# Chuanming-Liu/DAzimSurfTomo

Measured on AMD Instinct MI355X. Metric: FMM traveltime fields/sec (256^2 grid, 16 periods) + LSQR SpMV HBM GB/s, higher is better.
Workload: dtype f32

## Files before the change

dazimsurftomo_amd/csrc/disp.hip:

```cpp
#include <cmath>

#include "dazim_internal.h"

namespace {

constexpr int NL = 200;
constexpr int NP = 60;
constexpr int NZMAX = 64;
constexpr int DT = 256;
constexpr int TW = 64;
constexpr int TEAM = 16;
constexpr int NEVN = 11;

struct Layer {
  double tmp;
  float d;
  float rfac;
  float fm, den;
  int iv;
  float rden;
};

struct DispArgs {
  int ncol, nz, kmax, nvar, mmax;
  int team;
  int var0, nvarp;
  const float *vel;
  const Layer *lay;
  const double *t;
  float *cg;
  int ngroup, nchunk, pchunk;
  unsigned *counter;
  int *ready;
  double *st_c;
  double *st_d;
  int *st_f;
  int ffwd;
  int exp3;
  unsigned *ff_stat;
  int *ff_m;
  double *ff_c;
  int *ff_v;
  double *svs, *svp, *srho;
  double *pv;
  int *nfail;
};

__device__ __forceinline__ double sgn(double x) { return copysign(1.0, x); }

__device__ __forceinline__ double frcp(double b) {
  double r = __builtin_amdgcn_rcp(b);
  r = __builtin_fma(__builtin_fma(-b, r, 1.0), r, r);
  r = __builtin_fma(__builtin_fma(-b, r, 1.0), r, r);
  return r;
}
__device__ __forceinline__ double fdiv(double a, double b) {
  const double r = frcp(b);
  const double q = a * r;
  return __builtin_fma(__builtin_fma(-b, q, a), r, q);
}

__device__ __forceinline__ double fsqrt(double x, double &rs) {
  const double y = __builtin_amdgcn_rsq(x);
  double g = x * y, h = 0.5 * y;
  double r = __builtin_fma(-h, g, 0.5);
  g = __builtin_fma(g, r, g);
  h = __builtin_fma(h, r, h);
  r = __builtin_fma(-g, g, x);
  g = __builtin_fma(r, h, g);
  r = __builtin_fma(-h, g, 0.5);
  h = __builtin_fma(h, r, h);
  rs = h + h;
  return x > 0.0 ? g : 0.0;
}

struct Knots {
  const float *vs, *vp, *rho;
  int pi, pq;
  float pv;
  __device__ __forceinline__ float get(int q, int i) const {
    const float *b = q == 0 ? vs : (q == 1 ? vp : rho);
    const float v = b[i - 1];
    return (i == pi && q == pq) ? pv : v;
  }
};

template <int RDEN>
__device__ __forceinline__ void layer_model(const Knots &K, const Layer *lay, int m, int nz, bool fast, float &a,
                                            float &b, float &rho, float &d) {
  const Layer L = lay[m - 1];
  float rvp, rvs, rrho;
  if (L.iv > 0) {
    const int i = L.iv;
    const float p0 = K.get(1, i), p1 = K.get(1, i + 1);
    const float s0 = K.get(0, i), s1 = K.get(0, i + 1);
    const float r0 = K.get(2, i), r1 = K.get(2, i + 1);
    if (RDEN == 1) {
      rvp = p0 + L.fm * (p1 - p0) * L.rden;
      rvs = s0 + L.fm * (s1 - s0) * L.rden;
      rrho = r0 + L.fm * (r1 - r0) * L.rden;
    } else if (RDEN == 2 && fast) {
      const float tp = L.fm * (p1 - p0), ts = L.fm * (s1 - s0), tr = L.fm * (r1 - r0);
      float qp = tp * L.rden, qs = ts * L.rden, qr = tr * L.rden;
      qp = __builtin_fmaf(__builtin_fmaf(-L.den, qp, tp), L.rden, qp);
      qs = __builtin_fmaf(__builtin_fmaf(-L.den, qs, ts), L.rden, qs);
      qr = __builtin_fmaf(__builtin_fmaf(-L.den, qr, tr), L.rden, qr);
      rvp = p0 + qp;
      rvs = s0 + qs;
      rrho = r0 + qr;
    } else {
      rvp = p0 + L.fm * (p1 - p0) / L.den;
      rvs = s0 + L.fm * (s1 - s0) / L.den;
      rrho = r0 + L.fm * (r1 - r0) / L.den;
    }
  } else {
    rvp = K.get(1, nz);
    rvs = K.get(0, nz);
    rrho = K.get(2, nz);
  }
  a = (float)((double)rvp * L.tmp);
  b = (float)((double)rvs * L.tmp);
  rho = rrho * L.rfac;
  d = L.d;
}

template <int RDEN>
__device__ double dltar4(const Knots &K, const Layer *lay, int mmax, int nz, bool fast, double wvno, double omga, bool exp3 = false) {
#pragma clang fp contract(fast)
  double e0, e1, e2, e3, e4;
  double omega = omga;
  if (omega < 1.0e-4) omega = 1.0e-4;
  const double wvno2 = wvno * wvno;
  const double romega = 1.0 / omega;
  float fa, fb, frho, fd;
  layer_model<RDEN>(K, lay, mmax, nz, fast, fa, fb, frho, fd);
  {
    const double xka = omega / (double)fa, xkb = omega / (double)fb;
    double wvnop = wvno + xka, wvnom = fabs(wvno - xka);
    const double ra = sqrt(wvnop * wvnom);
    wvnop = wvno + xkb;
    wvnom = fabs(wvno - xkb);
    const double rb = sqrt(wvnop * wvnom);
    const double t = (double)fb / omega;
    const double gammk = 2.0 * t * t;
    const double gam = gammk * wvno2;
    const double gamm1 = gam - 1.0;
    const double rho1 = (double)frho;
    e0 = rho1 * rho1 * (gamm1 * gamm1 - gam * gammk * ra * rb);
    e1 = -rho1 * ra;
    e2 = rho1 * (gamm1 - gammk * ra * rb);
    e3 = rho1 * rb;
    e4 = wvno2 - ra * rb;
  }
  for (int m = mmax - 1; m >= 1; m--) {
    layer_model<RDEN>(K, lay, m, nz, fast, fa, fb, frho, fd);
    const double xka = fdiv(omega, (double)fa), xkb = fdiv(omega, (double)fb);
    const double t = (double)fb * romega;
    const double gammk = 2.0 * t * t;
    const double gam = gammk * wvno2;
    double wvnop = wvno + xka, wvnom = fabs(wvno - xka);
    double rra;
    const double ra = fsqrt(wvnop * wvnom, rra);
    wvnop = wvno + xkb;
    wvnom = fabs(wvno - xkb);
    double rrb;
    const double rb = fsqrt(wvnop * wvnom, rrb);
    const double dpth = (double)fd, rho1 = (double)frho;
    const double rrho1 = frcp(rho1), rrho2 = rrho1 * rrho1;
    const double p = ra * dpth, q = rb * dpth;
    double w, x, y, z, cosp, cosq, sinp, sinq, fac, pex = 0.0, sex = 0.0;
    if (wvno > xka) pex = p;
    if (wvno > xkb) sex = q;
    const double ep = pex > 0.0 ? exp(-pex) : 1.0, eq = sex > 0.0 ? exp(-sex) : 1.0;
    if (wvno < xka) {
      sincos(p, &sinp, &cosp);
      w = sinp * rra;
      x = -ra * sinp;
    } else if (wvno == xka) {
      cosp = 1.0;
      w = dpth;
      x = 0.0;
    } else {
      fac = 0.0;
      if (p < 16) fac = exp3 ? exp(-2.0 * p) : ep * ep;
      cosp = (1.0 + fac) * 0.5;
      sinp = (1.0 - fac) * 0.5;
      w = sinp * rra;
      x = ra * sinp;
    }
    if (wvno < xkb) {
      sincos(q, &sinq, &cosq);
      y = sinq * rrb;
      z = -rb * sinq;
    } else if (wvno == xkb) {
      cosq = 1.0;
      y = dpth;
      z = 0.0;
    } else {
      fac = 0.0;
      if (q < 16) fac = exp3 ? exp(-2.0 * q) : eq * eq;
      cosq = (1.0 + fac) * 0.5;
      sinq = (1.0 - fac) * 0.5;
      y = sinq * rrb;
      z = rb * sinq;
    }
    const double exa = pex + sex;
    double a0 = 0.0;
    if (exa < 60.0) a0 = exp3 ? exp(-exa) : ep * eq;
    const double cpcq = cosp * cosq, cpy = cosp * y, cpz = cosp * z, cqw = cosq * w, cqx = cosq * x;
    const double xy = x * y, xz = x * z, wy = w * y, wz = w * z;
    const double gamm1 = gam - 1.0;
    const double twgm1 = gam + gamm1, gmgmk = gam * gammk, gmgm1 = gam * gamm1, gm1sq = gamm1 * gamm1;
    const double rho2 = rho1 * rho1, a0pq = a0 - cpcq;
    const double ca11 = cpcq - 2.0 * gmgm1 * a0pq - gmgmk * xz - wvno2 * gm1sq * wy;
    const double ca12 = (wvno2 * cpy - cqx) * rrho1;
    const double ca13 = -(twgm1 * a0pq + gammk * xz + wvno2 * gamm1 * wy) * rrho1;
    const double ca14 = (cpz - wvno2 * cqw) * rrho1;
    const double ca15 = -(2.0 * wvno2 * a0pq + xz + wvno2 * wvno2 * wy) * rrho2;
    const double ca21 = (gmgmk * cpz - gm1sq * cqw) * rho1;
    const double ca22 = cpcq;
    const double ca23 = gammk * cpz - gamm1 * cqw;
    const double ca24 = -wz;
    const double ca25 = ca14;
    const double ca41 = (gm1sq * cpy - gmgmk * cqx) * rho1;
    const double ca42 = -xy;
    const double ca43 = gamm1 * cpy - gammk * cqx;
    const double ca44 = ca22;
    const double ca45 = ca12;
    const double ca51 = -(2.0 * gmgmk * gm1sq * a0pq + gmgmk * gmgmk * xz + gm1sq * gm1sq * wy) * rho2;
    const double ca52 = ca41;
    const double ca53 = -(gammk * gamm1 * twgm1 * a0pq + gam * gammk * gammk * xz + gamm1 * gm1sq * wy) * rho1;
    const double ca54 = ca21;
    const double ca55 = ca11;
    const double tt = -2.0 * wvno2;
    const double ca31 = tt * ca53, ca32 = tt * ca43, ca33 = a0 + 2.0 * (cpcq - ca11), ca34 = tt * ca23,
                 ca35 = tt * ca13;
    double n0 = 0.0 + e0 * ca11;  n0 = n0 + e1 * ca21;  n0 = n0 + e2 * ca31;  n0 = n0 + e3 * ca41;  n0 = n0 + e4 * ca51;
    double n1 = 0.0 + e0 * ca12;  n1 = n1 + e1 * ca22;  n1 = n1 + e2 * ca32;  n1 = n1 + e3 * ca42;  n1 = n1 + e4 * ca52;
    double n2 = 0.0 + e0 * ca13;  n2 = n2 + e1 * ca23;  n2 = n2 + e2 * ca33;  n2 = n2 + e3 * ca43;  n2 = n2 + e4 * ca53;
    double n3 = 0.0 + e0 * ca14;  n3 = n3 + e1 * ca24;  n3 = n3 + e2 * ca34;  n3 = n3 + e3 * ca44;  n3 = n3 + e4 * ca54;
    double n4 = 0.0 + e0 * ca15;  n4 = n4 + e1 * ca25;  n4 = n4 + e2 * ca35;  n4 = n4 + e3 * ca45;  n4 = n4 + e4 * ca55;
    double t1 = fmax(fmax(fmax(fabs(n0), fabs(n1)), fmax(fabs(n2), fabs(n3))), fabs(n4));
    if (t1 < 1.e-40) t1 = 1.0;
    const double r1 = frcp(t1);
    e0 = n0 * r1;
    e1 = n1 * r1;
    e2 = n2 * r1;
    e3 = n3 * r1;
    e4 = n4 * r1;
  }
  return e0;
}

__device__ float gtsolh(float a, float b) {
  float c = 0.95f * b;
  for (int i = 0; i < 5; i++) {
    const float gamma = b / a;
    const float kappa = c / b;
    const float k2 = kappa * kappa;
    const float gk2 = (gamma * kappa) * (gamma * kappa);
    const float fac1 = sqrtf(1.0f - gk2);
    const float fac2 = sqrtf(1.0f - k2);
    const float fr = (2.0f - k2) * (2.0f - k2) - 4.0f * fac1 * fac2;
    float frp = -4.0f * (2.0f - k2) * kappa + 4.0f * fac2 * gamma * gamma * kappa / fac1 + 4.0f * fac1 * kappa / fac2;
    frp = frp / b;
    c = c - fr / frp;
  }
  return c;
}

__device__ __forceinline__ void brocher(float vs, float &vp, float &rho) {
  const float v2 = vs * vs, v3 = v2 * vs, v4 = v3 * vs;
  const float p = 0.9409f + 2.0947f * vs - 0.8206f * v2 + 0.2683f * v3 - 0.0251f * v4;
  const float p2 = p * p, p3 = p2 * p, p4 = p3 * p, p5 = p4 * p;
  vp = p;
  rho = 1.6612f * p - 0.4721f * p2 + 0.0671f * p3 - 0.0043f * p4 + 0.000106f * p5;
}

enum { P_G1, P_G2, P_N0, P_NA, P_NB, P_GV, P_GW, P_DONE };

template <int RDEN>
__device__ __forceinline__ void startup(const Knots &K, const Layer *lay, int mmax, int nz, bool fast, float &betmx, float &cc1) {
  float betmn = 1.e20f, a_mn = 1.0f, b_mn = 1.0f;
  betmx = -1.e20f;
  int jsol = 1;
  for (int m = 1; m <= mmax; m++) {
    float fa, fb, fr, fd;
    layer_model<RDEN>(K, lay, m, nz, fast, fa, fb, fr, fd);
    if (fb > 0.01f && fb < betmn) {
      betmn = fb;
      a_mn = fa;
      b_mn = fb;
      jsol = 1;
    } else if (fb <= 0.01f && fa < betmn) {
      betmn = fa;
      a_mn = fa;
      b_mn = fb;
      jsol = 0;
    }
    if (fb > betmx) betmx = fb;
  }
  cc1 = jsol == 0 ? betmn : gtsolh(a_mn, b_mn);
  cc1 = .95f * cc1;
  cc1 = .90f * cc1;
}

constexpr int FF_BLOCKS = 8;
constexpr double FF_MARGIN = 0.02;
constexpr float FF_MAXDROP = 0.25f;
template <int RDEN>
__global__ __launch_bounds__(64) void disp_bracket_kernel(DispArgs A) {
  __shared__ Layer s_lay[NL];
  __shared__ float s_knot[3 * NZMAX];
  const int lane = threadIdx.x, col = blockIdx.x;
  const int nz = A.nz, mmax = A.mmax;
  for (int i = lane; i < mmax; i += 64) s_lay[i] = A.lay[i];
  for (int k = lane; k < nz; k += 64) {
    const float vs = A.vel[(size_t)k * A.ncol + col];
    float vp, rho;
    brocher(vs, vp, rho);
    s_knot[k] = vs;
    s_knot[nz + k] = vp;
    s_knot[2 * nz + k] = rho;
  }
  __syncthreads();
  Knots K;
  K.vs = s_knot;
  K.vp = s_knot + nz;
  K.rho = s_knot + 2 * nz;
  K.pi = 0;
  K.pq = -1;
  K.pv = 0.0f;
  bool fast = false;
  if (RDEN == 2) {
    bool ok = true;
    for (int i = 1; i < nz; i++)
#pragma unroll
      for (int q = 0; q < 3; q++) {
        const float ad = fabsf(K.get(q, i + 1) - K.get(q, i));
        ok = ok && (ad == 0.0f || (ad >= 1.0e-30f && ad <= 1.0e28f));
      }
    fast = __all(ok);
  }
  float betmx, cc1;
  startup<RDEN>(K, s_lay, mmax, nz, fast, betmx, cc1);
  const double dc = fabs((double)0.005f), TWOPI = 2.0 * 3.141592653589793;
  const double omega = TWOPI / A.t[0];
  const double climit = (double)betmx + dc;
  double cblk = (double)cc1;
  unsigned long long prev_last = 0;
  int found = 0;
  double cfound = 0.0, clast_prev = 0.0;
  double alast_prev = 0.0;
  int jfirst = -1;
  bool wiggle = false;
  for (int blk = 0; blk < FF_BLOCKS; blk++) {
    double c = cblk;
    for (int i = 0; i < lane; i++) c = c + dc;
    const double del = dltar4<RDEN>(K, s_lay, mmax, nz, fast, omega / c, omega, A.exp3 != 0);
    const unsigned long long neg = __ballot(sgn(del) < 0.0);
    const unsigned long long before = (neg << 1) | (blk > 0 ? prev_last : (neg & 1ull));
    const unsigned long long chg = neg ^ before;
    const unsigned long long over = __ballot(c >= climit);
    const int jl = over ? __builtin_ctzll(over) : 64;
    const double clast = __shfl(c, 63);
    {
      const double a = fabs(del);
      double ap = __shfl_up(a, 1);
      if (lane == 0) ap = blk > 0 ? alast_prev : a;
      const int jend = (chg != 0 && __builtin_ctzll(chg) <= jl) ? __builtin_ctzll(chg) : 64;
      const unsigned long long below = jend >= 64 ? ~0ull : ((1ull << jend) - 1ull);
      const unsigned long long dec = __ballot(a < ap * (1.0 - 1.0e-6)) & below;
      const unsigned long long inc = __ballot(a > ap * (1.0 + 1.0e-6)) & below;
      unsigned long long after = ~0ull;
      if (jfirst < 0 && dec != 0) {
        const int jd = __builtin_ctzll(dec);
        jfirst = 64 * blk + jd;
        after = jd >= 63 ? 0ull : ~((2ull << jd) - 1ull);
      } else if (jfirst < 0) {
        after = 0ull;
      }
      if ((inc & after) != 0) wiggle = true;
      alast_prev = __shfl(a, 63);
    }
    if (chg != 0) {
      const int j = __builtin_ctzll(chg);
      const double cl = __shfl(c, j > 0 ? j - 1 : 0);
      if (j <= jl) {
        found = 64 * blk + j;
        cfound = j > 0 ? cl : clast_prev;
      }
      break;
    }
    if (over != 0) break;
    prev_last = neg >> 63;
    clast_prev = clast;
    cblk = clast + dc;
  }
  if (lane == 0) {
    A.ff_m[col] = found > 0 ? found - 1 : 0;
    A.ff_c[col] = cfound;
    float vtop = s_knot[0], drop = 0.0f;
    for (int k = 1; k < nz; k++) {
      const float v = s_knot[k];
      drop = fmaxf(drop, (vtop - v) / vtop);
      vtop = fmaxf(vtop, v);
    }
    int lim = wiggle ? (jfirst - 8 > 0 ? jfirst - 8 : 0) : 0x3fffffff;
    if (drop > FF_MAXDROP) lim = 0;
    A.ff_v[col] = lim;
    if (A.ffwd == 2) {
      if (drop > FF_MAXDROP) atomicAdd(&A.ff_stat[0], 1u);
      else if (wiggle) atomicAdd(&A.ff_stat[1], 1u);
    }
  }
}

#ifdef DZ_DISP_STAT
__device__ unsigned long long g_disp_stat[4];
#endif
template <int RDEN, bool TEAMS = false>
__global__ __launch_bounds__(DT, 3) void disp_kernel(DispArgs A) {
  __shared__ Layer s_lay[NL];
  __shared__ double s_t[NP];
  extern __shared__ __attribute__((aligned(16))) float s_knots[];
  __shared__ double s_x[NEVN][DT], s_y[NEVN][DT];
  const int tid = threadIdx.x, lane = tid & 63;
  const int nz = A.nz, kmax = A.kmax, mmax = A.mmax, nvar = A.nvar, nvarp = A.nvarp;
  const long nwork = (long)A.ncol * nvarp;
  for (int i = tid; i < mmax; i += DT) s_lay[i] = A.lay[i];
  for (int i = tid; i < kmax; i += DT) s_t[i] = A.t[i];
  __syncthreads();
  const int team = TEAMS ? TEAM : 1, tw = TW / team;
  const int tl = lane & (team - 1), tsh = lane & ~(team - 1);
  const int cpb = (tw + nvarp - 1) / nvarp + 1;
  float *s_knot = s_knots + (size_t)(tid >> 6) * cpb * 3 * nz;
  const unsigned ntask = (unsigned)A.ngroup * (unsigned)A.nchunk;
  for (;;) {
    __builtin_amdgcn_wave_barrier();
    unsigned task = 0;
    if (lane == 0) {
      task = atomicAdd(A.counter, 1u);
      if (task < ntask && task >= (unsigned)A.ngroup) {
        const int *flag = A.ready + (task - (unsigned)A.ngroup);
        while (__hip_atomic_load(flag, __ATOMIC_ACQUIRE, __HIP_MEMORY_SCOPE_AGENT) == 0) __builtin_amdgcn_s_sleep(20);
      }
    }
    task = (unsigned)__shfl((int)task, 0);
    if (task >= ntask) break;
    __threadfence();
    const int chunk = (int)(task / (unsigned)A.ngroup), grp = (int)(task - (unsigned)chunk * (unsigned)A.ngroup);
    const int kbeg = chunk * A.pchunk, kend = min(kbeg + A.pchunk, kmax);
    const long w0 = (long)grp * tw;
    const int col0 = (int)(w0 / nvarp);
    for (int i = lane; i < cpb * nz; i += TW) {
      const int c = i / nz, k = i - c * nz, col = col0 + c;
      if (col < A.ncol) {
        const float vs = A.vel[(size_t)k * A.ncol + col];
        float vp, rho;
        brocher(vs, vp, rho);
        s_knot[(c * 3 + 0) * nz + k] = vs;
        s_knot[(c * 3 + 1) * nz + k] = vp;
        s_knot[(c * 3 + 2) * nz + k] = rho;
      }
    }
    __builtin_amdgcn_wave_barrier();
    const long w = w0 + (team > 1 ? lane / team : lane);
    const bool active = w < nwork;
    const int col = active ? (int)(w / nvarp) : col0;
    const int var = active ? A.var0 + (int)(w - (long)col * nvarp) : 0;
    Knots K;
    K.vs = s_knot + ((col - col0) * 3 + 0) * nz;
    K.vp = s_knot + ((col - col0) * 3 + 1) * nz;
    K.rho = s_knot + ((col - col0) * 3 + 2) * nz;
    K.pi = 0;
    K.pq = -1;
    K.pv = 0.0f;
    if (var > 0) {
      const int v1 = var - 1;
      K.pi = v1 / 6 + 1;
      const int r = v1 - (K.pi - 1) * 6;
      K.pq = r >> 1;
      const float b0 = (K.pq == 0 ? K.vs : (K.pq == 1 ? K.vp : K.rho))[K.pi - 1];
      const float dln = 0.01f;
      K.pv = (r & 1) ? b0 + 0.5f * dln * b0 : b0 - 0.5f * dln * b0;
    }
    bool fast = false;
    if (RDEN == 2) {
      bool ok = true;
      for (int i = 1; i < nz; i++)
#pragma unroll
        for (int q = 0; q < 3; q++) {
          const float ad = fabsf(K.get(q, i + 1) - K.get(q, i));
          ok = ok && (ad == 0.0f || (ad >= 1.0e-30f && ad <= 1.0e28f));
        }
      fast = __all(ok);
    }
    float betmx, cc1;
    startup<RDEN>(K, s_lay, mmax, nz, fast, betmx, cc1);
    const float ddc = 0.005f, sone = 1.5f;
    const double onea = (double)sone, TWOPI = 2.0 * 3.141592653589793;
    const double cc = (double)cc1, dc = fabs((double)ddc), cm = cc;
    const size_t wi = active ? (size_t)col * nvar + var : 0;
    float *cg = A.cg + wi * kmax;

    int k = kbeg, phase = active ? P_G1 : P_DONE, ifirst = 1, idir = 1, nev = 1, nctrl = 1, mm = 1;
    double c1 = cc, c2 = cc, del1 = 0, del2 = 0, del1st = 0, clow = cc, c3 = cc, del3 = 0, cprev = cc;
    if (chunk > 0 && active) {
      if (A.st_f[wi]) {
        phase = P_DONE;
      } else {
        cprev = A.st_c[wi];
        del1st = A.st_d[wi];
        ifirst = 0;
        c1 = cprev - onea * dc;
        clow = cm;
      }
    }
    double omega = TWOPI / s_t[kbeg];
    double ceval = c1;
    bool failed = false;
    double wc1 = 0.0, wc2 = 0.0;
    int wid = 1;

#ifdef DZ_DISP_STAT
    unsigned long long st_iter = 0, st_act = 0;
#endif
    while (__any(phase != P_DONE)) {
#ifdef DZ_DISP_STAT
      st_iter++;
      if (phase != P_DONE) st_act++;
#endif
      const double del = dltar4<RDEN>(K, s_lay, mmax, nz, fast, omega / ceval, omega, A.exp3 != 0);
      if (phase == P_DONE) continue;
      bool advance_bracket = false, nev_top = false, nev_body = false, finish = false, fail = false;
      switch (phase) {
        case P_G1:
          del1 = del;
          if (ifirst == 1) del1st = del1;
          idir = (ifirst == 1) ? 1 : (sgn(del1st) * sgn(del1) >= 0.0 ? 1 : -1);
          advance_bracket = true;
          if (A.ffwd && ifirst == 1 && chunk == 0) {
            int m = A.ff_m[col];
            if (var > 0 && A.ffwd < 2) m = 0;
            if (m > 0 && var > 0) {
              const double steps = floor((A.ff_c[col] - FF_MARGIN - c1) / dc);
              m = steps > 0.0 ? (steps < (double)m + 8.0 ? (int)steps : m + 8) : 0;
              const int lim = A.ff_v[col] - 4;
              if (m > lim) m = lim > 0 ? lim : 0;
            }
            if (m >= 2) {
              s_x[0][tid] = c1;
              for (int i = 0; i < m; i++) c1 = c1 + dc;
              ceval = c1;
              phase = P_GV;
              advance_bracket = false;
              if (var > 0) atomicAdd(&A.ff_stat[2], 1u);
            }
          }
          break;
        case P_GV:
          if (sgn(del) == sgn(del1))
            del1 = del;
          else {
            c1 = s_x[0][tid];
            if (var > 0) atomicAdd(&A.ff_stat[3], 1u);
          }
          advance_bracket = true;
          break;
        case P_G2:
          del2 = del;
          if (sgn(del1) != sgn(del2)) {
            c3 = 0.5 * (c1 + c2);
            ceval = c3;
            phase = P_N0;
            nev = 1;
            nctrl = 1;
            mm = 1;
          } else {
            c1 = c2;
            del1 = del2;
            if (c1 < cm || c1 >= ((double)betmx + dc))
              fail = true;
            else
              advance_bracket = true;
          }
          break;
        case P_GW: if (TEAMS) {
          const unsigned neg = (unsigned)(__ballot(sgn(del) < 0.0) >> tsh) & ((1u << TEAM) - 1u);
          const unsigned prevneg = ((neg << 1) | (sgn(del1) < 0.0 ? 1u : 0u)) & ((1u << TEAM) - 1u);
          const unsigned chg = neg ^ prevneg;
          const unsigned bad = (unsigned)(__ballot(wc2 < cm || wc2 >= ((double)betmx + dc)) >> tsh) & ((1u << TEAM) - 1u);
          const int jchg = chg ? __builtin_ctz(chg) : TEAM, jbad = bad ? __builtin_ctz(bad) : TEAM;
          if (jchg < TEAM && jchg <= jbad) {
            const double dprev = __shfl(del, tsh + (jchg > 0 ? jchg - 1 : 0));
            if (jchg > 0) del1 = dprev;
            c1 = __shfl(wc1, tsh + jchg);
            c2 = __shfl(wc2, tsh + jchg);
            del2 = __shfl(del, tsh + jchg);
            idir = __shfl(wid, tsh + jchg);
            c3 = 0.5 * (c1 + c2);
            ceval = c3;
            phase = P_N0;
            nev = 1;
            nctrl = 1;
            mm = 1;
          } else if (jbad < TEAM) {
            c1 = __shfl(wc2, tsh + jbad);
            fail = true;
          } else {
            c1 = __shfl(wc2, tsh + TEAM - 1);
            del1 = __shfl(del, tsh + TEAM - 1);
            idir = __shfl(wid, tsh + TEAM - 1);
            advance_bracket = true;
          }
        }
          break;
        case P_N0:
        case P_NB:
          del3 = del;
          nev_top = true;
          break;
        case P_NA:
          del3 = del;
          nev_body = true;
          break;
      }
      if (TEAMS && advance_bracket) {
        double a = c1;
        int id = idir;
        for (int i = 0; i <= tl; i++) {
          for (;;) {
            wc2 = (id > 0) ? a + dc : a - dc;
            if (wc2 <= clow) {
              id = 1;
              a = clow;
              continue;
            }
            break;
          }
          wc1 = a;
          a = wc2;
        }
        wid = id;
        ceval = wc2;
        phase = P_GW;
      } else if (!TEAMS && advance_bracket) {
        for (;;) {
          c2 = (idir > 0) ? c1 + dc : c1 - dc;
          if (c2 <= clow) {
            idir = 1;
            c1 = clow;
            continue;
          }
          break;
        }
        ceval = c2;
        phase = P_G2;
      }
      if (nev_top) {
        nctrl++;
        if (nctrl >= 100)
          finish = true;
        else if (c3 < fmin(c1, c2) || c3 > fmax(c1, c2)) {
          nev = 0;
          c3 = 0.5 * (c1 + c2);
          ceval = c3;
          phase = P_NA;
        } else
          nev_body = true;
      }
      if (nev_body) {
        const double s13 = del1 - del3, s32 = del3 - del2;
        if (sgn(del3) * sgn(del1) < 0.0) {
          c2 = c3;
          del2 = del3;
        } else {
          c1 = c3;
          del1 = del3;
        }
        if (fabs(c1 - c2) <= 1.e-6 * c1)
          finish = true;
        else {
          if (sgn(s13) != sgn(s32)) nev = 0;
          const double ss1 = fabs(del1), s1 = (double)0.01f * ss1;
          const double ss2 = fabs(del2), s2 = (double)0.01f * ss2;
          if (s1 > ss2 || s2 > ss1 || nev == 0) {
            c3 = 0.5 * (c1 + c2);
            nev = 1;
            mm = 1;
          } else {
            if (nev == 2) {
              s_x[mm][tid] = c3;
              s_y[mm][tid] = del3;
            } else {
              s_x[0][tid] = c1;
              s_y[0][tid] = del1;
              s_x[1][tid] = c2;
              s_y[1][tid] = del2;
              mm = 1;
            }
            bool bad = false;
            const double ym = s_y[mm][tid];
            for (int kk = 1; kk <= mm; kk++) {
              const int j = mm - kk + 1;
              const double yj = s_y[j - 1][tid];
              const double denom = ym - yj;
              if (fabs(denom) < 1.0e-10 * fabs(ym)) {
                bad = true;
                break;
              }
              s_x[j - 1][tid] = (-yj * s_x[j][tid] + ym * s_x[j - 1][tid]) / denom;
            }
            if (!bad) {
              c3 = s_x[0][tid];
              nev = 2;
              mm = mm + 1;
              if (mm > 10) mm = 10;
            } else {
              c3 = 0.5 * (c1 + c2);
              nev = 1;
              mm = 1;
            }
          }
          ceval = c3;
          phase = P_NB;
        }
      }
      if (finish) {
        c1 = c3;
        if (c1 > (double)betmx)
          fail = true;
        else {
          cg[k] = (float)c1;
          cprev = c1;
          k++;
          if (k == kend)
            phase = P_DONE;
          else {
            ifirst = 0;
            c1 = cprev - onea * dc;
            clow = cm;
            omega = TWOPI / s_t[k];
            ceval = c1;
            phase = P_G1;
          }
        }
      }
      if (fail) {
        for (int i = k; i < kmax; i++) cg[i] = 0.0f;
        failed = true;
        phase = P_DONE;
      }
    }
#ifdef DZ_DISP_STAT
    {
      atomicAdd(&g_disp_stat[0], st_act);
      if (lane == 0) { atomicAdd(&g_disp_stat[1], st_iter * 64ull); atomicAdd(&g_disp_stat[2], st_iter * 64ull); }
    }
#endif
    if (A.pv && kend == kmax && active && var == 0 && tl == 0) {
      int nzero = 0;
      for (int kk = 0; kk < kmax; kk++) {
        const float c0 = cg[kk];
        A.pv[(size_t)kk * A.ncol + col] = (double)c0;
        nzero += c0 == 0.0f ? 1 : 0;
      }
      if (nzero) atomicAdd(A.nfail, nzero);
    }
    if (A.svs && kend == kmax && team == 1) {
      double *const out = K.pq == 0 ? A.svs : (K.pq == 1 ? A.svp : A.srho);
      const float base = active && var > 0 ? (K.pq == 0 ? K.vs : (K.pq == 1 ? K.vp : K.rho))[K.pi - 1] : 1.0f;
      const double den = (double)(0.01f * base);
      for (int kk = 0; kk < kmax; kk++) {
        const float mine = active ? cg[kk] : 0.0f;
        const float other = __shfl_xor(mine, 1);
        if (active && !(lane & 1)) out[((size_t)(K.pi - 1) * kmax + kk) * A.ncol + col] = ((double)other - (double)mine) / den;
      }
    }
    if (active && kend < kmax && !(chunk > 0 && A.st_f[wi])) {
      A.st_c[wi] = cprev;
      A.st_d[wi] = del1st;
      A.st_f[wi] = failed ? 1 : 0;
    }
    __threadfence();
    __builtin_amdgcn_wave_barrier();
    if (lane == 0 && kend < kmax) __hip_atomic_store(A.ready + task, 1, __ATOMIC_RELEASE, __HIP_MEMORY_SCOPE_AGENT);
  }
}

__global__ void disp_finalize(int ncol, int nz, int kmax, int nvar, const float *__restrict__ vel,
                              const float *__restrict__ cg, double *__restrict__ pv, double *__restrict__ svs,
                              double *__restrict__ svp, double *__restrict__ srho, int *nfail) {
  const long tid = (long)blockIdx.x * blockDim.x + threadIdx.x;
  if (tid >= (long)ncol * kmax) return;
  const int k = (int)(tid / ncol), col = (int)(tid - (long)k * ncol);
  const float *c = cg + (size_t)col * nvar * kmax;
  if (pv) {
    const float c0 = c[k];
    pv[(size_t)k * ncol + col] = (double)c0;
    if (c0 == 0.0f) atomicAdd(nfail, 1);
  }
  if (!svs) return;
  const float dln = 0.01f;
  for (int i = 0; i < nz; i++) {
    const float vs = vel[(size_t)i * ncol + col];
    float vp, rho;
    brocher(vs, vp, rho);
    const float base[3] = {vs, vp, rho};
    double *out[3] = {svs, svp, srho};
    for (int q = 0; q < 3; q++) {
      const float cg1 = c[(size_t)(1 + i * 6 + q * 2) * kmax + k], cg2 = c[(size_t)(1 + i * 6 + q * 2 + 1) * kmax + k];
      out[q][((size_t)i * kmax + k) * ncol + col] = ((double)cg2 - (double)cg1) / (double)(dln * base[q]);
    }
  }
}

}

extern "C" int dazim_dispersion_kernels(dazim_ctx *ctx, int nx, int ny, int nz, const float *vel_u,
                                        const float *depz, float minthk0, int kmax, const double *periods,
                                        double *pv_u, double *svs_u, double *svp_u, double *srho_u, int *n_failed) {
  if (!ctx || !vel_u || !depz || !periods || !pv_u) return dz_fail(ctx, DAZIM_E_BAD_ARG, "null argument");
  if (nz < 2 || nz > NZMAX || kmax < 1 || kmax > NP || nx < 1 || ny < 1) return dz_fail(ctx, DAZIM_E_BAD_ARG, "bad nz/kmax");
  DZ_HIP(hipSetDevice(ctx->device));
  const bool kernels = svs_u && svp_u && srho_u;
  const int ncol = nx * ny, nvar = kernels ? 1 + 6 * nz : 1;
  std::vector<Layer> lay;
  for (int i = 1; i <= nz - 1; i++) {
    const float thk = depz[i] - depz[i - 1];
    const float minthk = thk / minthk0;
    const int nsub = (int)((thk + 1.0e-4f) / minthk) + 1;
    const float newthk = thk / (float)nsub;
    for (int j = 1; j <= nsub; j++) {
      Layer L;
      L.d = newthk;
      L.iv = i;
      L.fm = (float)(2 * j - 1);
      L.den = (float)(2 * nsub);
      lay.push_back(L);
    }
  }
  {
    Layer L;
    L.d = 0.0f;
    L.iv = 0;
    L.fm = 0;
    L.den = 1;
    lay.push_back(L);
  }
  int rden = 1;
  for (Layer &L : lay) {
    const int d = (int)L.den;
    L.rden = 1.0f / L.den;
    const bool pow2 = (d & (d - 1)) == 0 && d <= (1 << 20);
    bool fastdiv_ok = false;
    for (int v : {6, 10, 12, 14, 18, 20, 22, 24, 26, 28, 30, 36}) fastdiv_ok = fastdiv_ok || d == v;
    if (!pow2) rden = (fastdiv_ok && rden != 0) ? 2 : 0;
  }
  if (ctx->opts.count("disp.rden") && !ctx->opts["disp.rden"]) rden = 0;
  const int mmax = (int)lay.size();
  if (mmax > NL) return dz_fail(ctx, DAZIM_E_BAD_ARG, "refined model has %d layers > NL=%d", mmax, NL);
  {
    const double ar = 6370.0;
    double dr = 0.0, r0 = ar;
    lay[mmax - 1].d = 1.0f;
    for (int i = 0; i < mmax; i++) {
      dr = dr + (double)lay[i].d;
      const double r1 = ar - dr;
      const double z0 = ar * log(ar / r0), z1 = ar * log(ar / r1);
      lay[i].d = (float)(z1 - z0);
      const double tmp = (ar + ar) / (r0 + r1);
      lay[i].tmp = tmp;
      lay[i].rfac = powf((float)tmp, -2.275f);
      r0 = r1;
    }
    lay[mmax - 1].d = 0.0f;
  }
  DzBuf<float> vel;
  DzBuf<double> pv, svs, svp, srho;
  int rc;
  if ((rc = dz_fmm_finish(ctx))) return rc;
  if ((rc = dz_join_aux(ctx))) return rc;
  const size_t nk = (size_t)nz * kmax * ncol;
  if ((rc = vel.init(ctx, vel_u, (size_t)nz * ncol, true, false))) return rc;
  if ((rc = pv.init(ctx, pv_u, (size_t)kmax * ncol, false, true))) return rc;
  if (kernels) {
    if ((rc = svs.init(ctx, svs_u, nk, false, true))) return rc;
    if ((rc = svp.init(ctx, svp_u, nk, false, true))) return rc;
    if ((rc = srho.init(ctx, srho_u, nk, false, true))) return rc;
  }
  void *p;
  DispArgs A;
  A.svs = A.svp = A.srho = A.pv = nullptr;
  A.nfail = nullptr;
  A.ncol = ncol;
  A.nz = nz;
  A.kmax = kmax;
  A.nvar = nvar;
  A.var0 = 0;
  A.nvarp = nvar;
  A.team = 1;
  A.mmax = mmax;
  A.vel = vel.dev;
  if ((rc = dz_scratch(ctx, "disp.lay", sizeof(Layer) * NL, &p))) return rc;
  A.lay = (Layer *)p;
  DZ_HIP(hipMemcpyAsync(p, lay.data(), sizeof(Layer) * mmax, hipMemcpyHostToDevice, ctx->stream));
  if ((rc = dz_scratch(ctx, "disp.t", sizeof(double) * NP, &p))) return rc;
  A.t = (double *)p;
  DZ_HIP(hipMemcpyAsync(p, periods, sizeof(double) * kmax, hipMemcpyHostToDevice, ctx->stream));
  if ((rc = dz_scratch(ctx, "disp.cg", sizeof(float) * (size_t)ncol * nvar * kmax, &p))) return rc;
  A.cg = (float *)p;
  if ((rc = dz_scratch(ctx, "disp.nfail", 16, &p))) return rc;
  int *d_nfail = (int *)p;
  DZ_HIP(hipMemsetAsync(d_nfail, 0, 4, ctx->stream));
  DZ_HIP(hipStreamSynchronize(ctx->stream));
  auto knot_lds = [&](int nvarp, int items = TW) { return (size_t)(DT / TW) * ((items + nvarp - 1) / nvarp + 1) * 3 * nz * sizeof(float); };
  bool async = kernels && ctx->opts.count("disp.async") && ctx->opts["disp.async"] && !vel.staged && !svs.staged &&
               !svp.staged && !srho.staged && !(ctx->opts.count("disp.pchunk") && ctx->opts["disp.pchunk"] > 0 && ctx->opts["disp.pchunk"] < kmax);
  const double wg_copies = (double)(((long)ncol * (nvar - 1) + DT - 1) / DT), wg_teams = (double)((ncol * TEAM + DT - 1) / DT);
  const double wg_round = (double)((long)ctx->num_cu * 3);
  bool teams = wg_copies + wg_teams <= 0.98 * wg_round || (wg_copies > 1.02 * wg_round && wg_copies + wg_teams <= 1.9 * wg_round);
  if (ctx->opts.count("disp.team") && ctx->opts["disp.team"] == 1) teams = true;
  if (ctx->opts.count("disp.team") && ctx->opts["disp.team"] == 2) teams = false;
  const size_t dyn_lds = knot_lds(nvar), dyn_lds_base = teams ? knot_lds(1, TW / TEAM) : knot_lds(1);
  if (dyn_lds_base + 56 * 1024 > 160 * 1024) async = false;
  const size_t dyn_max = async && dyn_lds_base > dyn_lds ? dyn_lds_base : dyn_lds;
  DZ_HIP(hipFuncSetAttribute((const void *)disp_kernel<0>, hipFuncAttributeMaxDynamicSharedMemorySize, (int)dyn_max));
  DZ_HIP(hipFuncSetAttribute((const void *)disp_kernel<1>, hipFuncAttributeMaxDynamicSharedMemorySize, (int)dyn_max));
  DZ_HIP(hipFuncSetAttribute((const void *)disp_kernel<2>, hipFuncAttributeMaxDynamicSharedMemorySize, (int)dyn_max));
  DZ_HIP(hipFuncSetAttribute((const void *)disp_kernel<0, true>, hipFuncAttributeMaxDynamicSharedMemorySize, (int)dyn_max));
  DZ_HIP(hipFuncSetAttribute((const void *)disp_kernel<1, true>, hipFuncAttributeMaxDynamicSharedMemorySize, (int)dyn_max));
  DZ_HIP(hipFuncSetAttribute((const void *)disp_kernel<2, true>, hipFuncAttributeMaxDynamicSharedMemorySize, (int)dyn_max));
  if (async && (rc = dz_aux_init(ctx))) return rc;
  {
    const long nwork = (long)ncol * nvar;
    A.ngroup = (int)((nwork + TW - 1) / TW);
    A.pchunk = kmax;
    if (ctx->opts.count("disp.pchunk") && ctx->opts["disp.pchunk"] > 0) A.pchunk = ctx->opts["disp.pchunk"];
    if (A.pchunk > kmax) A.pchunk = kmax;
    A.nchunk = (kmax + A.pchunk - 1) / A.pchunk;
    const size_t ntask = (size_t)A.ngroup * A.nchunk;
    if ((rc = dz_scratch(ctx, "disp.ready", ntask * 4 + 64, &p))) return rc;
    A.ready = (int *)p;
    A.counter = (unsigned *)((char *)p + ntask * 4 + 16 - (ntask * 4) % 16);
    DZ_HIP(hipMemsetAsync(p, 0, ntask * 4 + 64, ctx->stream));
    if ((rc = dz_scratch(ctx, "disp.st_c", (size_t)nwork * 8, &p))) return rc;
    A.st_c = (double *)p;
    if ((rc = dz_scratch(ctx, "disp.st_d", (size_t)nwork * 8, &p))) return rc;
    A.st_d = (double *)p;
    if ((rc = dz_scratch(ctx, "disp.st_f", (size_t)nwork * 4, &p))) return rc;
    A.st_f = (int *)p;
    const void *kf = rden == 1 ? (const void *)disp_kernel<1> : (rden == 2 ? (const void *)disp_kernel<2> : (const void *)disp_kernel<0>);
    int occ = 3;
    if (hipOccupancyMaxActiveBlocksPerMultiprocessor(&occ, kf, DT, dyn_lds) != hipSuccess || occ < 1) occ = 1;
    long nwg = (long)ctx->num_cu * occ;
    if (nwg > ((long)ntask + DT / TW - 1) / (DT / TW)) nwg = ((long)ntask + DT / TW - 1) / (DT / TW);
    A.ffwd = 0;
    if (A.nchunk == 1) {
      A.ffwd = 1;
      if (ctx->opts.count("disp.ffwd")) A.ffwd = ctx->opts["disp.ffwd"] < 0 ? 0 : (ctx->opts["disp.ffwd"] > 2 ? 2 : ctx->opts["disp.ffwd"]);
    }
    A.exp3 = ctx->opts.count("disp.exp3") && ctx->opts["disp.exp3"] ? 1 : 0;
    if ((rc = dz_scratch(ctx, "disp.ff_stat", 64, &p))) return rc;
    A.ff_stat = (unsigned *)p;
    DZ_HIP(hipMemsetAsync(A.ff_stat, 0, 64, ctx->stream));
    if ((rc = dz_scratch(ctx, "disp.ff_m", (size_t)ncol * 4 + 16, &p))) return rc;
    A.ff_m = (int *)p;
    if ((rc = dz_scratch(ctx, "disp.ff_c", (size_t)ncol * 8 + 16, &p))) return rc;
    A.ff_c = (double *)p;
    if ((rc = dz_scratch(ctx, "disp.ff_v", (size_t)ncol * 4 + 16, &p))) return rc;
    A.ff_v = (int *)p;
    if (async && ctx->opts["disp.async"] == 1) {
      const double rounds = (double)(((long)ncol * (nvar - 1) + DT - 1) / DT) / (double)((long)ctx->num_cu * occ);
      if (rounds > 2.0) async = false;
    }
    ctx->ksec["disp.async"] = async ? 1.0 : 0.0;
    ctx->aux_timed = false;
    DzTimer t(ctx, "disp");
    if (A.ffwd) {
      if (rden == 1)
        hipLaunchKernelGGL(disp_bracket_kernel<1>, dim3((unsigned)ncol), dim3(64), 0, ctx->stream, A);
      else if (rden == 2)
        hipLaunchKernelGGL(disp_bracket_kernel<2>, dim3((unsigned)ncol), dim3(64), 0, ctx->stream, A);
      else
        hipLaunchKernelGGL(disp_bracket_kernel<0>, dim3((unsigned)ncol), dim3(64), 0, ctx->stream, A);
      DZ_HIP(hipGetLastError());
    }
    auto launch = [&](const DispArgs &B, long nwgB, size_t lds, hipStream_t st) {
      if (B.team > 1) {
        if (rden == 1)
          hipLaunchKernelGGL((disp_kernel<1, true>), dim3((unsigned)nwgB), dim3(DT), lds, st, B);
        else if (rden == 2)
          hipLaunchKernelGGL((disp_kernel<2, true>), dim3((unsigned)nwgB), dim3(DT), lds, st, B);
        else
          hipLaunchKernelGGL((disp_kernel<0, true>), dim3((unsigned)nwgB), dim3(DT), lds, st, B);
      } else if (rden == 1)
        hipLaunchKernelGGL(disp_kernel<1>, dim3((unsigned)nwgB), dim3(DT), lds, st, B);
      else if (rden == 2)
        hipLaunchKernelGGL(disp_kernel<2>, dim3((unsigned)nwgB), dim3(DT), lds, st, B);
      else
        hipLaunchKernelGGL(disp_kernel<0>, dim3((unsigned)nwgB), dim3(DT), lds, st, B);
    };
    const long nf = (long)ncol * kmax;
    if (!async) {
      launch(A, nwg, dyn_lds, ctx->stream);
      DZ_HIP(hipGetLastError());
      hipLaunchKernelGGL(disp_finalize, dim3((unsigned)((nf + 255) / 256)), dim3(256), 0, ctx->stream, ncol, nz, kmax, nvar,
                         vel.dev, A.cg, pv.dev, kernels ? svs.dev : nullptr, kernels ? svp.dev : nullptr,
                         kernels ? srho.dev : nullptr, d_nfail);
      DZ_HIP(hipGetLastError());
    } else {
      DispArgs C = A;
      C.var0 = 1;
      C.nvarp = nvar - 1;
      C.ngroup = (int)(((long)ncol * C.nvarp + TW - 1) / TW);
      long nwgC = (long)ctx->num_cu * occ, needC = ((long)C.ngroup + DT / TW - 1) / (DT / TW);
      if (nwgC > needC) nwgC = needC;
      DispArgs B = A;
      B.var0 = 0;
      B.nvarp = 1;
      B.team = teams ? TEAM : 1;
      B.pv = pv.dev;
      B.nfail = d_nfail;
      B.ngroup = (ncol + TW / B.team - 1) / (TW / B.team);
      ctx->ksec["disp.team"] = B.team;
      if ((rc = dz_scratch(ctx, "disp.ready_b", (size_t)B.ngroup * 4 + 64, &p))) return rc;
      B.ready = (int *)p;
      B.counter = (unsigned *)((char *)p + (size_t)B.ngroup * 4 + 16 - ((size_t)B.ngroup * 4) % 16);
      DZ_HIP(hipMemsetAsync(p, 0, (size_t)B.ngroup * 4 + 64, ctx->stream));
      DZ_HIP(hipEventRecord(ctx->ev_fork, ctx->stream));
      const long nwgB = ((long)B.ngroup + DT / TW - 1) / (DT / TW);
      launch(B, nwgB, dyn_lds_base, ctx->stream);
      DZ_HIP(hipGetLastError());
      DZ_HIP(hipStreamWaitEvent(ctx->stream2, ctx->ev_fork, 0));
      DZ_HIP(hipEventRecord(ctx->ev_a0, ctx->stream2));
      C.svs = svs.dev;
      C.svp = svp.dev;
      C.srho = srho.dev;
      launch(C, nwgC, dyn_lds, ctx->stream2);
      DZ_HIP(hipGetLastError());
      DZ_HIP(hipEventRecord(ctx->ev_a1, ctx->stream2));
      ctx->aux_pending = true;
      ctx->aux_timed = true;
      ctx->aux_ranges.clear();
      ctx->aux_ranges.push_back({(const char *)vel.dev, (size_t)nz * ncol * sizeof(float)});
      for (const double *q : {svs.dev, svp.dev, srho.dev})
        if (q) ctx->aux_ranges.push_back({(const char *)q, nk * sizeof(double)});
    }
    t.stop();
  }
  if ((rc = dz_pinned(ctx, "disp.host", 64, &p))) return rc;
  int &nfail = *(int *)p;
  unsigned *hst = (unsigned *)p + 4;
  nfail = 0;
  hst[0] = hst[1] = hst[2] = hst[3] = 0;
  DZ_HIP(hipMemcpyAsync(&nfail, d_nfail, 4, hipMemcpyDeviceToHost, ctx->stream));
#ifdef DZ_DISP_STAT
  {
    unsigned long long h[4];
    DZ_HIP(hipMemcpyFromSymbol(h, HIP_SYMBOL(g_disp_stat), sizeof h));
    fprintf(stderr, "disp stat: lane-evaluations done %llu, offered by the wavefronts %llu (%.3f used), by the workgroups %llu (%.3f used)\n", h[0], h[1],
            (double)h[0] / (double)h[1], h[2], (double)h[0] / (double)h[2]);
    unsigned long long z[4] = {0};
    DZ_HIP(hipMemcpyToSymbol(HIP_SYMBOL(g_disp_stat), z, sizeof z));
  }
#endif
  if (!ctx->aux_pending) DZ_HIP(hipMemcpyAsync(hst, A.ff_stat, 16, hipMemcpyDeviceToHost, ctx->stream));
  if ((rc = pv.finish()) || (rc = svs.finish()) || (rc = svp.finish()) || (rc = srho.finish())) return rc;
  DZ_HIP(hipStreamSynchronize(ctx->stream));
  if (n_failed) *n_failed = nfail;
  ctx->ksec["disp.ffwd_mode"] = A.ffwd;
  ctx->ksec["disp.ffwd_gated_columns"] = hst[0];
  ctx->ksec["disp.ffwd_dip_columns"] = hst[1];
  ctx->ksec["disp.ffwd_jumped_copies"] = hst[2];
  ctx->ksec["disp.ffwd_fallback_copies"] = hst[3];
  return 0;
}
```

Before: 53420.

## Precompute per-column layer tables in LDS and patch perturbed layers per lane

Instead of re-evaluating layer_model interpolation for every layer inside each dltar4 call, the dispersion kernels now precompute a per-column table of layer (vp, vs, rho, d) values in shared memory. Each lane adds a small patch covering only the layers affected by its perturbed knot, computed from a host-side krange table. To free the LDS this needs, the Neville interpolation scratch moves to a global buffer. This trades extra LDS and global traffic for removing repeated interpolation arithmetic in the hot determinant loop, and it may lower occupancy.

```diff
diff --git a/dazimsurftomo_amd/csrc/disp.hip b/dazimsurftomo_amd/csrc/disp.hip
--- a/dazimsurftomo_amd/csrc/disp.hip
+++ b/dazimsurftomo_amd/csrc/disp.hip
@@ -1,3 +1,4 @@
+#include <algorithm>
 #include <cmath>
 
 #include "dazim_internal.h"
@@ -44,6 +45,9 @@
   double *svs, *svp, *srho;
   double *pv;
   int *nfail;
+  int npatch;
+  const int *krange;
+  double *nev;
 };
 
 __device__ __forceinline__ double sgn(double x) { return copysign(1.0, x); }
@@ -125,7 +129,35 @@
 }
 
 template <int RDEN>
-__device__ double dltar4(const Knots &K, const Layer *lay, int mmax, int nz, bool fast, double wvno, double omga, bool exp3 = false) {
+struct KnotLayers {
+  const Knots &K;
+  const Layer *lay;
+  int nz;
+  bool fast;
+  __device__ __forceinline__ void get(int m, float &a, float &b, float &rho, float &d) const {
+    layer_model<RDEN>(K, lay, m, nz, fast, a, b, rho, d);
+  }
+};
+template <bool PATCH>
+struct TableLayers {
+  const float *lds;
+  int boff;
+  int poff;
+  int m_lo;
+  unsigned cnt;
+  __device__ __forceinline__ void get(int m, float &a, float &b, float &rho, float &d) const {
+    const int ib = boff + 4 * m;
+    int i = ib;
+    if (PATCH) i = (unsigned)(m - m_lo) < cnt ? poff + 3 * TW * m : ib;
+    a = lds[i];
+    b = lds[i + 1];
+    rho = lds[i + 2];
+    d = lds[ib + 3];
+  }
+};
+
+template <class LS>
+__device__ double dltar4(const LS &S, int mmax, double wvno, double omga, bool exp3 = false) {
 #pragma clang fp contract(fast)
   double e0, e1, e2, e3, e4;
   double omega = omga;
@@ -133,7 +165,7 @@
   const double wvno2 = wvno * wvno;
   const double romega = 1.0 / omega;
   float fa, fb, frho, fd;
-  layer_model<RDEN>(K, lay, mmax, nz, fast, fa, fb, frho, fd);
+  S.get(mmax, fa, fb, frho, fd);
   {
     const double xka = omega / (double)fa, xkb = omega / (double)fb;
     double wvnop = wvno + xka, wvnom = fabs(wvno - xka);
@@ -153,7 +185,7 @@
     e4 = wvno2 - ra * rb;
   }
   for (int m = mmax - 1; m >= 1; m--) {
-    layer_model<RDEN>(K, lay, m, nz, fast, fa, fb, frho, fd);
+    S.get(m, fa, fb, frho, fd);
     const double xka = fdiv(omega, (double)fa), xkb = fdiv(omega, (double)fb);
     const double t = (double)fb * romega;
     const double gammk = 2.0 * t * t;
@@ -279,14 +311,14 @@
 
 enum { P_G1, P_G2, P_N0, P_NA, P_NB, P_GV, P_GW, P_DONE };
 
-template <int RDEN>
-__device__ __forceinline__ void startup(const Knots &K, const Layer *lay, int mmax, int nz, bool fast, float &betmx, float &cc1) {
+template <class LS>
+__device__ __forceinline__ void startup(const LS &S, int mmax, float &betmx, float &cc1) {
   float betmn = 1.e20f, a_mn = 1.0f, b_mn = 1.0f;
   betmx = -1.e20f;
   int jsol = 1;
   for (int m = 1; m <= mmax; m++) {
     float fa, fb, fr, fd;
-    layer_model<RDEN>(K, lay, m, nz, fast, fa, fb, fr, fd);
+    S.get(m, fa, fb, fr, fd);
     if (fb > 0.01f && fb < betmn) {
       betmn = fb;
       a_mn = fa;
@@ -312,6 +344,7 @@
 __global__ __launch_bounds__(64) void disp_bracket_kernel(DispArgs A) {
   __shared__ Layer s_lay[NL];
   __shared__ float s_knot[3 * NZMAX];
+  __shared__ float4 s_base[NL];
   const int lane = threadIdx.x, col = blockIdx.x;
   const int nz = A.nz, mmax = A.mmax;
   for (int i = lane; i < mmax; i += 64) s_lay[i] = A.lay[i];
@@ -342,8 +375,15 @@
       }
     fast = __all(ok);
   }
+  for (int m = lane + 1; m <= mmax; m += 64) {
+    float a, b, r, d;
+    layer_model<RDEN>(K, s_lay, m, nz, fast, a, b, r, d);
+    s_base[m - 1] = make_float4(a, b, r, d);
+  }
+  __syncthreads();
+  const TableLayers<false> S{(const float *)s_base, -4, 0, 0, 0u};
   float betmx, cc1;
-  startup<RDEN>(K, s_lay, mmax, nz, fast, betmx, cc1);
+  startup(S, mmax, betmx, cc1);
   const double dc = fabs((double)0.005f), TWOPI = 2.0 * 3.141592653589793;
   const double omega = TWOPI / A.t[0];
   const double climit = (double)betmx + dc;
@@ -357,7 +397,7 @@
   for (int blk = 0; blk < FF_BLOCKS; blk++) {
     double c = cblk;
     for (int i = 0; i < lane; i++) c = c + dc;
-    const double del = dltar4<RDEN>(K, s_lay, mmax, nz, fast, omega / c, omega, A.exp3 != 0);
+    const double del = dltar4(S, mmax, omega / c, omega, A.exp3 != 0);
     const unsigned long long neg = __ballot(sgn(del) < 0.0);
     const unsigned long long before = (neg << 1) | (blk > 0 ? prev_last : (neg & 1ull));
     const unsigned long long chg = neg ^ before;
@@ -419,12 +459,18 @@
 #ifdef DZ_DISP_STAT
 __device__ unsigned long long g_disp_stat[4];
 #endif
-template <int RDEN, bool TEAMS = false>
+template <int RDEN, bool TEAMS = false, bool SHARE = false>
 __global__ __launch_bounds__(DT, 3) void disp_kernel(DispArgs A) {
+  static_assert(!(TEAMS && SHARE), "a team holds one item: nothing to share");
   __shared__ Layer s_lay[NL];
   __shared__ double s_t[NP];
   extern __shared__ __attribute__((aligned(16))) float s_knots[];
-  __shared__ double s_x[NEVN][DT], s_y[NEVN][DT];
+  constexpr int NEVL = SHARE ? 1 : DT;
+  __shared__ double s_x[NEVN][NEVL], s_y[NEVN][NEVL];
+  const size_t nev_n = (size_t)gridDim.x * DT;
+  double *const nev_x = SHARE ? A.nev + (size_t)blockIdx.x * DT + threadIdx.x : nullptr, *const nev_y = SHARE ? nev_x + NEVN * nev_n : nullptr;
+  auto NX = [&](int i) -> double & { if constexpr (SHARE) return nev_x[(size_t)i * nev_n]; else return s_x[i][threadIdx.x]; };
+  auto NY = [&](int i) -> double & { if constexpr (SHARE) return nev_y[(size_t)i * nev_n]; else return s_y[i][threadIdx.x]; };
   const int tid = threadIdx.x, lane = tid & 63;
   const int nz = A.nz, kmax = A.kmax, mmax = A.mmax, nvar = A.nvar, nvarp = A.nvarp;
   const long nwork = (long)A.ncol * nvarp;
@@ -496,8 +542,37 @@
         }
       fast = __all(ok);
     }
+    const KnotLayers<RDEN> SK{K, s_lay, nz, fast};
+    TableLayers<true> ST{s_knots, 0, 0, 0, 0u};
+    if constexpr (SHARE) {
+      float4 *const s_tab = (float4 *)(s_knots + (((DT / TW) * cpb * 3 * nz + 3) & ~3));
+      float4 *const s_base = s_tab + (size_t)(tid >> 6) * cpb * mmax;
+      float *const s_patch = (float *)(s_tab + (size_t)(DT / TW) * cpb * mmax) + (size_t)(tid >> 6) * A.npatch * 3 * TW + 3 * lane;
+      ST.boff = (int)((const float *)(s_base + (size_t)(col - col0) * mmax) - s_knots) - 4;
+      for (int i = lane; i < cpb * mmax; i += TW) {
+        const int c = i / mmax, m = i - c * mmax + 1;
+        if (col0 + c >= A.ncol) continue;
+        const Knots Kc{s_knot + (c * 3 + 0) * nz, s_knot + (c * 3 + 1) * nz, s_knot + (c * 3 + 2) * nz, 0, -1, 0.0f};
+        float a, b, r, d;
+        layer_model<RDEN>(Kc, s_lay, m, nz, fast, a, b, r, d);
+        s_base[i] = make_float4(a, b, r, d);
+      }
+      ST.m_lo = A.krange[2 * K.pi];
+      ST.cnt = (unsigned)A.krange[2 * K.pi + 1];
+      ST.poff = (int)(s_patch - s_knots) - 3 * TW * ST.m_lo;
+      for (unsigned j = 0; j < (unsigned)A.npatch; j++)
+        if (j < ST.cnt) {
+          float a, b, r, d;
+          layer_model<RDEN>(K, s_lay, ST.m_lo + (int)j, nz, fast, a, b, r, d);
+          s_patch[j * (3 * TW) + 0] = a;
+          s_patch[j * (3 * TW) + 1] = b;
+          s_patch[j * (3 * TW) + 2] = r;
+        }
+      __builtin_amdgcn_wave_barrier();
+    }
     float betmx, cc1;
-    startup<RDEN>(K, s_lay, mmax, nz, fast, betmx, cc1);
+    if constexpr (SHARE) startup(ST, mmax, betmx, cc1);
+    else startup(SK, mmax, betmx, cc1);
     const float ddc = 0.005f, sone = 1.5f;
     const double onea = (double)sone, TWOPI = 2.0 * 3.141592653589793;
     const double cc = (double)cc1, dc = fabs((double)ddc), cm = cc;
@@ -531,7 +606,9 @@
       st_iter++;
       if (phase != P_DONE) st_act++;
 #endif
-      const double del = dltar4<RDEN>(K, s_lay, mmax, nz, fast, omega / ceval, omega, A.exp3 != 0);
+      double del;
+      if constexpr (SHARE) del = dltar4(ST, mmax, omega / ceval, omega, A.exp3 != 0);
+      else del = dltar4(SK, mmax, omega / ceval, omega, A.exp3 != 0);
       if (phase == P_DONE) continue;
       bool advance_bracket = false, nev_top = false, nev_body = false, finish = false, fail = false;
       switch (phase) {
@@ -550,7 +627,7 @@
               if (m > lim) m = lim > 0 ? lim : 0;
             }
             if (m >= 2) {
-              s_x[0][tid] = c1;
+              NX(0) = c1;
               for (int i = 0; i < m; i++) c1 = c1 + dc;
               ceval = c1;
               phase = P_GV;
@@ -563,7 +640,7 @@
           if (sgn(del) == sgn(del1))
             del1 = del;
           else {
-            c1 = s_x[0][tid];
+            c1 = NX(0);
             if (var > 0) atomicAdd(&A.ff_stat[3], 1u);
           }
           advance_bracket = true;
@@ -691,29 +768,29 @@
             mm = 1;
           } else {
             if (nev == 2) {
-              s_x[mm][tid] = c3;
-              s_y[mm][tid] = del3;
+              NX(mm) = c3;
+              NY(mm) = del3;
             } else {
-              s_x[0][tid] = c1;
-              s_y[0][tid] = del1;
-              s_x[1][tid] = c2;
-              s_y[1][tid] = del2;
+              NX(0) = c1;
+              NY(0) = del1;
+              NX(1) = c2;
+              NY(1) = del2;
               mm = 1;
             }
             bool bad = false;
-            const double ym = s_y[mm][tid];
+            const double ym = NY(mm);
             for (int kk = 1; kk <= mm; kk++) {
               const int j = mm - kk + 1;
-              const double yj = s_y[j - 1][tid];
+              const double yj = NY(j - 1);
               const double denom = ym - yj;
               if (fabs(denom) < 1.0e-10 * fabs(ym)) {
                 bad = true;
                 break;
               }
-              s_x[j - 1][tid] = (-yj * s_x[j][tid] + ym * s_x[j - 1][tid]) / denom;
+              NX(j - 1) = (-yj * NX(j) + ym * NX(j - 1)) / denom;
             }
             if (!bad) {
-              c3 = s_x[0][tid];
+              c3 = NX(0);
               nev = 2;
               mm = mm + 1;
               if (mm > 10) mm = 10;
@@ -903,6 +980,23 @@
   A.team = 1;
   A.mmax = mmax;
   A.vel = vel.dev;
+  std::vector<int> krange(2 * (nz + 1), 0);
+  A.npatch = 1;
+  for (int pi = 1; pi <= nz; pi++) {
+    int lo = 0, hi = 0;
+    for (int m = 1; m <= mmax; m++)
+      if ((pi > 1 && lay[m - 1].iv == pi - 1) || lay[m - 1].iv == pi || (pi == nz && lay[m - 1].iv == 0)) {
+        if (!lo) lo = m;
+        hi = m;
+      }
+    krange[2 * pi] = lo;
+    krange[2 * pi + 1] = lo ? hi - lo + 1 : 0;
+    if (krange[2 * pi + 1] > A.npatch) A.npatch = krange[2 * pi + 1];
+  }
+  A.nev = nullptr;
+  if ((rc = dz_scratch(ctx, "disp.krange", sizeof(int) * 2 * (NZMAX + 1), &p))) return rc;
+  A.krange = (const int *)p;
+  DZ_HIP(hipMemcpyAsync(p, krange.data(), sizeof(int) * krange.size(), hipMemcpyHostToDevice, ctx->stream));
   if ((rc = dz_scratch(ctx, "disp.lay", sizeof(Layer) * NL, &p))) return rc;
   A.lay = (Layer *)p;
   DZ_HIP(hipMemcpyAsync(p, lay.data(), sizeof(Layer) * mmax, hipMemcpyHostToDevice, ctx->stream));
@@ -932,6 +1026,21 @@
   DZ_HIP(hipFuncSetAttribute((const void *)disp_kernel<0, true>, hipFuncAttributeMaxDynamicSharedMemorySize, (int)dyn_max));
   DZ_HIP(hipFuncSetAttribute((const void *)disp_kernel<1, true>, hipFuncAttributeMaxDynamicSharedMemorySize, (int)dyn_max));
   DZ_HIP(hipFuncSetAttribute((const void *)disp_kernel<2, true>, hipFuncAttributeMaxDynamicSharedMemorySize, (int)dyn_max));
+  const void *kshare = rden == 1 ? (const void *)disp_kernel<1, false, true>
+                                 : (rden == 2 ? (const void *)disp_kernel<2, false, true> : (const void *)disp_kernel<0, false, true>);
+  auto share_lds = [&](int nvarp) {
+    const size_t cpb = (size_t)(TW + nvarp - 1) / nvarp + 1, knots = (((size_t)(DT / TW) * cpb * 3 * nz + 3) & ~(size_t)3) * sizeof(float);
+    return knots + (size_t)(DT / TW) * cpb * mmax * sizeof(float4) + (size_t)(DT / TW) * A.npatch * 3 * TW * sizeof(float);
+  };
+  bool share = kernels && !(ctx->opts.count("disp.share") && !ctx->opts["disp.share"]);
+  if (share) {
+    hipFuncAttributes fa;
+    DZ_HIP(hipFuncGetAttributes(&fa, kshare));
+    const size_t need = std::max(share_lds(nvar), share_lds(nvar - 1));
+    share = fa.sharedSizeBytes + need <= (size_t)42 * 1280;
+    if (share) DZ_HIP(hipFuncSetAttribute(kshare, hipFuncAttributeMaxDynamicSharedMemorySize, (int)need));
+  }
+  ctx->ksec["disp.share"] = share ? 1.0 : 0.0;
   if (async && (rc = dz_aux_init(ctx))) return rc;
   {
     const long nwork = (long)ncol * nvar;
@@ -953,7 +1062,11 @@
     A.st_f = (int *)p;
     const void *kf = rden == 1 ? (const void *)disp_kernel<1> : (rden == 2 ? (const void *)disp_kernel<2> : (const void *)disp_kernel<0>);
     int occ = 3;
-    if (hipOccupancyMaxActiveBlocksPerMultiprocessor(&occ, kf, DT, dyn_lds) != hipSuccess || occ < 1) occ = 1;
+    if (hipOccupancyMaxActiveBlocksPerMultiprocessor(&occ, share ? kshare : kf, DT, share ? share_lds(nvar) : dyn_lds) != hipSuccess || occ < 1) occ = 1;
+    if (share) {
+      if ((rc = dz_scratch(ctx, "disp.nev", sizeof(double) * 2 * NEVN * (size_t)ctx->num_cu * occ * DT, &p))) return rc;
+      A.nev = (double *)p;
+    }
     long nwg = (long)ctx->num_cu * occ;
     if (nwg > ((long)ntask + DT / TW - 1) / (DT / TW)) nwg = ((long)ntask + DT / TW - 1) / (DT / TW);
     A.ffwd = 0;
@@ -988,7 +1101,15 @@
       DZ_HIP(hipGetLastError());
     }
     auto launch = [&](const DispArgs &B, long nwgB, size_t lds, hipStream_t st) {
-      if (B.team > 1) {
+      if (share && B.team == 1 && B.nvarp > 1) {
+        lds = share_lds(B.nvarp);
+        if (rden == 1)
+          hipLaunchKernelGGL((disp_kernel<1, false, true>), dim3((unsigned)nwgB), dim3(DT), lds, st, B);
+        else if (rden == 2)
+          hipLaunchKernelGGL((disp_kernel<2, false, true>), dim3((unsigned)nwgB), dim3(DT), lds, st, B);
+        else
+          hipLaunchKernelGGL((disp_kernel<0, false, true>), dim3((unsigned)nwgB), dim3(DT), lds, st, B);
+      } else if (B.team > 1) {
         if (rden == 1)
           hipLaunchKernelGGL((disp_kernel<1, true>), dim3((unsigned)nwgB), dim3(DT), lds, st, B);
         else if (rden == 2)
```

Measured after the change: 54340 (median of 6 runs). 1.7% higher.
